# mcychan/nQuant.android

Hardware: NVIDIA B200
Metric: Mpixels/s 256-color PNN quantize+dither, 4K batch, 1/2/4/8 B200 vs JVM CPU (higher is better)
Workload: dtype f64

## Files before the change

### include/nquant_b200.h

```cpp
#ifndef NQUANT_B200_H
#define NQUANT_B200_H

#include <stdint.h>

#ifdef __cplusplus
extern "C" {
#endif

#define NQ_KIND_PNN 0
#define NQ_KIND_PNNLAB 1

#define NQ_OK 0
#define NQ_ERR_CUDA (-1)
#define NQ_ERR_ARG (-2)
#define NQ_ERR_COLOR (-3)
#define NQ_ERR_UNSUPPORTED (-4)
#define NQ_ERR_NOMEM (-5)

typedef struct nq_ctx nq_ctx;

int nq_device_count(void);

nq_ctx* nq_create(int device);
void nq_destroy(nq_ctx* ctx);
// ... 15 lines not shown
int nq_convert_batch_multi(nq_ctx** contexts, int n_contexts, int kind, const uint32_t* argb_in, int n_images, int width, int height,
                           int n_max_colors, int dither, const uint64_t* rng_seeds, uint32_t* argb_out, uint32_t* palettes_out,
                           int* palette_lens, int* has_alpha, int queue_images);

int nq_convert_batch_device(nq_ctx* ctx, int kind, const uint32_t* d_argb_in, int n_images, int width, int height,
                            int n_max_colors, int dither, const uint64_t* rng_seeds, uint32_t* d_argb_out,
                            uint32_t* palettes_out, int* palette_lens, int* has_alpha);

int nq_dither_with_palette(nq_ctx* ctx, int kind, const uint32_t* argb_in, int width, int height, int n_max_colors,
                           int dither, uint64_t rng_seed, const uint32_t* palette_in, int palette_len, uint32_t* argb_out);

int nq_histogram(nq_ctx* ctx, int kind, const uint32_t* argb_in, int width, int height, int n_max_colors, int* n_bins,
                 double* bins5, float* init_err, int* init_nn, int capacity);

int nq_gilbert_order(int width, int height, uint32_t* order_out);


typedef struct nq_image_info {
  int has_semi_transparency;
  int transparent_pixel_index;
  uint32_t transparent_color;
  int maxbins, quan_rt, texicab, is_nano;
  double weight, ratio_init, ratio_merge, pr, pg, pb, pa;
  int g_margin, g_thresold, g_dither_max_q, g_dither_max, g_sorted, g_has_alpha, g_use_saliency;
  float g_beta;
  float bn_weight;
  int palette_len;
  unsigned long long merges, rescans, pair_tests, rng_draws, heap_pops;
  int error;
  unsigned long long full_evals;
  unsigned long long merge_cycles[6], live_blocks, screened;
  unsigned long long dither_cycles[3];
  unsigned long long merge_rounds, rescans_discarded;
} nq_image_info;
int nq_get_image_info(nq_ctx* ctx, int image, nq_image_info* out);
int nq_sizeof_image_info(void);

int nq_set_spec_dither(nq_ctx* ctx, int on, int segment, int warmup);
int nq_get_spec_stats(nq_ctx* ctx, unsigned long long* images, unsigned long long* rounds, unsigned long long* fallbacks);

int nq_set_debug(nq_ctx* ctx, int flag);
int nq_debug_get_bins(nq_ctx* ctx, int image, double* bins5, float* init_err, int* init_nn);
int nq_debug_get_merges(nq_ctx* ctx, int image, int* pairs);
int nq_debug_get_saliencies(nq_ctx* ctx, int image, float* out);

unsigned long long nq_kernel_launches(nq_ctx* ctx);
int nq_get_stage_times(nq_ctx* ctx, double* ms, unsigned long long* launches, int reset);
int nq_get_kernel_times(nq_ctx* ctx, double* ms, unsigned long long* launches, int reset);
int nq_debug_math(nq_ctx* ctx, int fn, const double* x, const double* y, double* out, int n);

int nq_debug_ciede(nq_ctx* ctx, const float* lab1, const float* lab2, float* out, int* n_exact, int n);

int nq_synth_device(nq_ctx* ctx, uint32_t* d_out, int n_images, int width, int height, int cls, int alpha_mode,
                    uint64_t seed0);

#ifdef __cplusplus
}
#endif
#endif
```

### nquant_android_b200/_lib.py

```python
import ctypes
import os

HERE = os.path.dirname(os.path.abspath(__file__))
SO = os.path.join(HERE, "libnquant_b200.so")

SYMBOLS = [
    "nq_device_count", "nq_create", "nq_destroy", "nq_last_error", "nq_convert", "nq_convert_batch",
    "nq_convert_batch_device", "nq_dither_with_palette", "nq_gilbert_order", "nq_get_image_info", "nq_set_debug",
    "nq_debug_get_bins", "nq_debug_get_merges", "nq_debug_get_saliencies", "nq_kernel_launches", "nq_debug_math",
    "nq_synth_device", "nq_get_stage_times", "nq_set_stream", "nq_debug_ciede", "nq_sizeof_image_info",
    "nq_set_spec_dither", "nq_get_spec_stats", "nq_reset_stream", "nq_set_chunk_images", "nq_get_kernel_times", "nq_convert_batch_multi", "nq_histogram",
]

NQ_KIND_PNN, NQ_KIND_PNNLAB = 0, 1
NQ_OK, NQ_ERR_CUDA, NQ_ERR_ARG, NQ_ERR_COLOR, NQ_ERR_UNSUPPORTED, NQ_ERR_NOMEM = 0, -1, -2, -3, -4, -5


class ImageInfo(ctypes.Structure):
    _fields_ = [
        ("has_semi_transparency", ctypes.c_int), ("transparent_pixel_index", ctypes.c_int),
        ("transparent_color", ctypes.c_uint32),
        ("maxbins", ctypes.c_int), ("quan_rt", ctypes.c_int), ("texicab", ctypes.c_int), ("is_nano", ctypes.c_int),
        ("weight", ctypes.c_double), ("ratio_init", ctypes.c_double), ("ratio_merge", ctypes.c_double),
        ("pr", ctypes.c_double), ("pg", ctypes.c_double), ("pb", ctypes.c_double), ("pa", ctypes.c_double),
        ("g_margin", ctypes.c_int), ("g_thresold", ctypes.c_int), ("g_dither_max_q", ctypes.c_int),
        ("g_dither_max", ctypes.c_int), ("g_sorted", ctypes.c_int), ("g_has_alpha", ctypes.c_int),
        ("g_use_saliency", ctypes.c_int),
        ("g_beta", ctypes.c_float), ("bn_weight", ctypes.c_float), ("palette_len", ctypes.c_int),
        ("merges", ctypes.c_ulonglong), ("rescans", ctypes.c_ulonglong), ("pair_tests", ctypes.c_ulonglong),
        ("rng_draws", ctypes.c_ulonglong), ("heap_pops", ctypes.c_ulonglong),
        ("error", ctypes.c_int),
        ("full_evals", ctypes.c_ulonglong),
        ("merge_cycles", ctypes.c_ulonglong * 6), ("live_blocks", ctypes.c_ulonglong), ("screened", ctypes.c_ulonglong),
        ("dither_cycles", ctypes.c_ulonglong * 3),
        ("merge_rounds", ctypes.c_ulonglong), ("rescans_discarded", ctypes.c_ulonglong),
    ]

    def as_dict(self):
        return {n: (list(getattr(self, n)) if n in ("merge_cycles", "dither_cycles") else getattr(self, n)) for n, _ in self._fields_}


_lib = None


def load():
    global _lib
    if _lib is not None:
        return _lib
    if not os.path.exists(SO):
        raise ImportError(f"{SO} is missing: run `python -c 'import __graft_entry__ as g; g.build()'` "
                          "(nvcc, sm_100a). This package has no CPU fallback.")
    L = ctypes.CDLL(SO)
    vp, ci, u64 = ctypes.c_void_p, ctypes.c_int, ctypes.c_uint64
    L.nq_device_count.restype = ci
    L.nq_create.restype = vp
    L.nq_create.argtypes = [ci]
    L.nq_destroy.argtypes = [vp]
    L.nq_destroy.restype = None
    L.nq_last_error.restype = ctypes.c_char_p
    L.nq_convert.argtypes = [vp, ci, vp, ci, ci, ci, ci, u64, vp, vp, vp, vp]
    L.nq_convert_batch.argtypes = [vp, ci, vp, ci, ci, ci, ci, ci, vp, vp, vp, vp, vp]
    L.nq_convert_batch_device.argtypes = [vp, ci, vp, ci, ci, ci, ci, ci, vp, vp, vp, vp, vp]
    L.nq_convert_batch_multi.argtypes = [vp, ci, ci, vp, ci, ci, ci, ci, ci, vp, vp, vp, vp, vp, ci]
    L.nq_dither_with_palette.argtypes = [vp, ci, vp, ci, ci, ci, ci, u64, vp, ci, vp]
    L.nq_gilbert_order.argtypes = [ci, ci, vp]
    L.nq_histogram.argtypes = [vp, ci, vp, ci, ci, ci, vp, vp, vp, vp, ci]
    L.nq_get_image_info.argtypes = [vp, ci, vp]
    L.nq_set_debug.argtypes = [vp, ci]
# ... 22 lines not shown
```

### nquant_android_b200/csrc/nq_api.cu

```cuda
#include <cuda_runtime.h>
#include <stdint.h>
#include <stdio.h>
#include <stdlib.h>
#include <string.h>
#include <string>
#include <vector>
#include <map>
#include <utility>
#include <algorithm>
#include <mutex>
#include <thread>
#include <atomic>
#include <nvtx3/nvToolsExt.h>

#include "../../include/nquant_b200.h"
#include "nq_types.h"
#include "nq_math.h"
#include "nq_color.h"
#include "nq_bluenoise_table.h"
#include "nq_hist.cuh"
#include "nq_pnn.cuh"
#include "nq_dither.cuh"
#include "nq_dither_spec.cuh"

// ... 116 lines not shown
  out[4 * i] = tL; out[4 * i + 1] = tC; out[4 * i + 2] = tH; out[4 * i + 3] = tRT;
}

__global__ void k_set_palette(NqImage* imgs, int img, const uint32_t* pal, int plen) {
  if (threadIdx.x < plen) imgs[img].palette[threadIdx.x] = pal[threadIdx.x];
  if (threadIdx.x == 0) imgs[img].paletteLen = plen;
}

struct LabLutEntry { float4* ptr = nullptr; int refs = 0; };
std::mutex g_lutMutex;
std::map<int, LabLutEntry> g_lut;

struct DebugImage {
  std::vector<double> bins5;
  std::vector<float> initErr;
  std::vector<int> initNn;
  std::vector<int> merges;
  std::vector<float> sal;
};

}

#define NQ_FRONT_STREAMS 2
#define NQ_SPEC_BULK_DEFAULT 0

struct nq_ctx {
  int device = 0;
  cudaStream_t stream = nullptr;
  cudaStream_t ownStream = nullptr;
  cudaStream_t sFront[NQ_FRONT_STREAMS] = {}, sDith = nullptr, sAux = nullptr, sOut = nullptr, sIn = nullptr;
  std::vector<cudaEvent_t> evPool;
  size_t evUsed = 0;
  int smCount = 148;
  unsigned long long launches = 0;
  bool debug = false;
  int chunkImages = 0;
  std::map<std::pair<int, int>, uint32_t*> orders;
  std::vector<std::pair<int, int>> orderLru;
  size_t orderBytes = 0;
  unsigned char* ws = nullptr;
  size_t wsBytes = 0;
  NqImage* dImgs = nullptr;
  NqSlot* dSlots = nullptr;
  int* dLive = nullptr;
  int* dPos = nullptr;
  unsigned char* zeroPlane = nullptr;
  unsigned char* memoPlane = nullptr;
  unsigned char* sortPool = nullptr;
  size_t zeroSlotBytes = 0, memoSlotBytes = 0, sortSetBytes = 0, sortABytes = 0;
  int wsSlots = 0, wsNpix = 0, wsKind = -1, sortSets = 0;
  bool wsDebug = false, wsBits = false, wsIdx = false;
  std::vector<NqSlot> hSlots;
  uint32_t* dIn = nullptr;
  uint32_t* dOut = nullptr;
  size_t stageBytes = 0;
  double stageMs[NQ_NSTAGES] = {};
  unsigned long long stageLaunches[NQ_NSTAGES] = {};
  double kernelMs[NQ_NKERNELS] = {};
  unsigned long long kernelLaunches[NQ_NKERNELS] = {};
  bool specDither = true;
  int specSeg = 0, specWarm = 1024;
  size_t specPoolMaxBytes = 0;
  int specSlotsMax = 0;
  nq::spec::SpecImage* dSpec = nullptr;
  int specCap = 0;
  unsigned char* specBuf = nullptr;
// ... 127 lines not shown
  uint32_t* d = nullptr;
  CU(cudaMalloc(&d, bytes));
  cudaError_t e = cudaMemcpy(d, host.data(), bytes, cudaMemcpyHostToDevice);
  if (e != cudaSuccess) { cudaFree(d); return fail(NQ_ERR_CUDA, std::string("cudaMemcpy(order): ") + cudaGetErrorString(e)); }
  c->orders[key] = d;
  c->orderLru.push_back(key);
  c->orderBytes += bytes;
  *out = d;
  return NQ_OK;
}

int pixel_grid_x(const nq_ctx* c, int npix, int nimg) {
  int want = (npix + 256 * 8 - 1) / (256 * 8);
  int cap = std::max(1, (c->smCount * 8) / std::max(1, nimg));
  return std::max(1, std::min(want, cap));
}

cudaEvent_t take_event(nq_ctx* c) {
  if (c->evUsed == c->evPool.size()) {
    cudaEvent_t e = nullptr;
    cudaEventCreate(&e);
    c->evPool.push_back(e);
  }
  return c->evPool[c->evUsed++];
}

struct NvtxRange {
  explicit NvtxRange(const char* name) { nvtxRangePushA(name); }
  ~NvtxRange() { nvtxRangePop(); }
};

struct Chunk {
  int base = 0, n = 0;
  cudaStream_t front = nullptr;
  int frontIdx = 0;
  cudaEvent_t evIn = nullptr;
  cudaEvent_t ev[5] = {};
  cudaEvent_t evD[3] = {};
  cudaEvent_t evK[2 * NQ_NKERNELS] = {};
  std::vector<std::pair<cudaEvent_t, cudaEvent_t>> evRuns;
  unsigned long long launches[NQ_NSTAGES] = {};
  int copied = 0;
  uint32_t* hOut = nullptr;
  const uint32_t* dOut = nullptr;
  size_t imageBytes = 0;
};

struct SpecCudaBackend {
  nq_ctx* c;
  Chunk* ch;
  cudaStream_t st;
  bool timing = false;
  cudaEvent_t t0 = nullptr, t1 = nullptr;
  cudaError_t err = cudaSuccess;
  template <class... P, class... A>
  void launch(void (*kernel)(P...), dim3 grid, int block, A... args) {
    kernel<<<grid, block, 0, st>>>(args...);
    ++c->launches;
  }
  template <class... P, class... A>
  void launch_run(void (*kernel)(P...), dim3 grid, int block, A... args) {
    cudaEvent_t a = take_event(c), b = take_event(c);
    cudaEventRecord(a, st);
    kernel<<<grid, block, 0, st>>>(args...);
    cudaEventRecord(b, st);
    ch->evRuns.emplace_back(a, b);
// ... 84 lines not shown
  for (int i = 0; i < n; ++i) plan->any += (elig[i] & 255) == 1;
  plan->seg = seg; plan->nslots = nslots;
  return NQ_OK;
}
int spec_rounds(nq_ctx* c, Chunk& ch, cudaStream_t st, int npix, const SpecPlan& plan, const std::vector<int>& elig, std::vector<int>& handed) {
  using namespace nq::spec;
  handed.clear();
  if (!plan.any) return NQ_OK;
  SpecCudaBackend be{c, &ch, st};
  be.timing = getenv("NQ_SPEC_TIMING") != nullptr;
  be.begin();
  SpecStats stats;
  handed.assign(plan.any, 0);
  spec_drive(be, c->dImgs + ch.base, c->dSpec + ch.base, c->dSpecPool, elig.data(), ch.n, npix, plan.seg, plan.nslots, c->dSpecInts, c->dTanh,
             c->smCount, &stats, handed.data());
  handed.resize((size_t)stats.handedBack);
  be.end();
  c->specImages += stats.done; c->specRounds += stats.rounds; c->specFallbacks += stats.handedBack;
  CU(be.err);
  CU(cudaGetLastError());
  return NQ_OK;
}

struct GroupArgs {
  int kind, w, h, nmax, dither;
  const uint64_t* seeds;
  const uint32_t* dPalIn;
  int palInLen;
  const uint32_t* hIn;
  uint32_t* hOut;
  bool stopAfterSweep = false;
};

int enqueue_front(nq_ctx* c, Chunk& ch, const GroupArgs& A, const uint32_t* dIn, uint32_t* dOut) {
  NvtxRange nv("nq front (scan, histogram, find_nn, merge)");
  const int n = ch.n, npix = A.w * A.h, kind = A.kind, nmax = A.nmax;
  cudaStream_t st = ch.front;
  NqImage* dI = c->dImgs + ch.base;
  NqSlot* dS = c->dSlots + ch.base;
  if (ch.evIn) CU(cudaStreamWaitEvent(st, ch.evIn, 0));
  std::vector<NqImage> hImgs(n);
  for (int i = 0; i < n; ++i) {
    NqImage& I = hImgs[i];
    memset(&I, 0, sizeof(I));
    I.kind = kind; I.width = A.w; I.height = A.h; I.npix = npix; I.nmax = nmax; I.dither = A.dither;
    I.seed = A.seeds ? A.seeds[ch.base + i] : 0ULL;
    I.transIdx = -1;
    NqSlot& S = c->hSlots[ch.base + i];
    S.in = dIn + (size_t)(ch.base + i) * npix;
    S.out = dOut + (size_t)(ch.base + i) * npix;
    if (kind == NQ_KIND_LAB) {
      unsigned char* sp = c->sortPool + c->sortSetBytes * ((size_t)ch.frontIdx * c->sortSets + (size_t)(i % c->sortSets));
      S.sortA = reinterpret_cast<uint32_t*>(sp);
      S.sortB = reinterpret_cast<uint32_t*>(sp + c->sortABytes);
      S.warpHist = reinterpret_cast<unsigned int*>(sp + 2 * c->sortABytes);
    }
  }
  CU(cudaMemcpyAsync(dI, hImgs.data(), sizeof(NqImage) * n, cudaMemcpyHostToDevice, st));
  CU(cudaMemcpyAsync(dS, c->hSlots.data() + ch.base, sizeof(NqSlot) * n, cudaMemcpyHostToDevice, st));
  CU(cudaMemsetAsync(c->zeroPlane + c->zeroSlotBytes * ch.base, 0, c->zeroSlotBytes * n, st));
  CU(cudaMemsetAsync(c->memoPlane + c->memoSlotBytes * ch.base, 0xFF, c->memoSlotBytes * n, st));
  for (int i = 0; i < n; ++i) if (c->hSlots[ch.base + i].bits) CU(cudaMemsetAsync(c->hSlots[ch.base + i].bits, 0, (size_t)1 << 29, st));
  const int gx = pixel_grid_x(c, npix, n);
  const dim3 pg(gx, n);
  unsigned long long l0 = c->launches;
  auto mark = [&](int k) { cudaEventRecord(ch.ev[k], st); if (k > 0) { ch.launches[k - 1] += c->launches - l0; l0 = c->launches; } };
  mark(0);
  nq::k_alpha_scan<<<pg, 256, 0, st>>>(dI, dS); ++c->launches;
  nq::k_setup_scan<<<(n + 127) / 128, 128, 0, st>>>(dI, dS, n); ++c->launches;
  mark(1);
  if (nmax > 2) {
    if (kind == NQ_KIND_RGB) {
      {
        const int ntiles = ((A.w + NQ_HTW - 1) / NQ_HTW) * ((A.h + NQ_HTW - 1) / NQ_HTW);
        const dim3 hg(std::max(1, std::min(ntiles, std::max(1, c->smCount * 8 / n))), n);
        nq::k_hist_rgb<<<hg, 256, sizeof(nq::HistTable), st>>>(dI, dS); ++c->launches;
      }
      nq::k_finalize_rgb<<<n, 1024, 0, st>>>(dI, dS); ++c->launches;
    } else {
      const int nruns = (npix + NQ_RUN - 1) / NQ_RUN;
// ... 30 lines not shown
      std::vector<NqImage> tmp(n);
      CU(cudaMemcpy(tmp.data(), dI, sizeof(NqImage) * n, cudaMemcpyDeviceToHost));
      for (int i = 0; i < n; ++i) {
        DebugImage& D = c->dbg[ch.base + i];
        const int mb = tmp[i].maxbins;
        const NqSlot& S = c->hSlots[ch.base + i];
        D.bins5.assign((size_t)mb * 5, 0.0);
        D.initErr.assign(mb, 0.f); D.initNn.assign(mb, 0);
        if (mb <= 0) continue;
        std::vector<double> col(mb);
        std::vector<float> colf(mb);
        for (int k = 0; k < 4; ++k) {
          if (kind == NQ_KIND_RGB) {
            const double* src = k == 0 ? S.bAc : k == 1 ? S.bC1 : k == 2 ? S.bC2 : S.bC3;
            CU(cudaMemcpy(col.data(), src, (size_t)mb * 8, cudaMemcpyDeviceToHost));
          } else {
            const float* src = k == 0 ? S.fAc : k == 1 ? S.fC1 : k == 2 ? S.fC2 : S.fC3;
            CU(cudaMemcpy(colf.data(), src, (size_t)mb * 4, cudaMemcpyDeviceToHost));
            for (int b = 0; b < mb; ++b) col[b] = colf[b];
          }
          for (int b = 0; b < mb; ++b) D.bins5[(size_t)b * 5 + k] = col[b];
        }
        CU(cudaMemcpy(colf.data(), S.bCnt, (size_t)mb * 4, cudaMemcpyDeviceToHost));
        for (int b = 0; b < mb; ++b) D.bins5[(size_t)b * 5 + 4] = colf[b];
        CU(cudaMemcpy(D.initErr.data(), S.bErr, (size_t)mb * 4, cudaMemcpyDeviceToHost));
        CU(cudaMemcpy(D.initNn.data(), S.bNn, (size_t)mb * 4, cudaMemcpyDeviceToHost));
      }
    }
    if (A.stopAfterSweep) { mark(4); CU(cudaGetLastError()); return NQ_OK; }
    int* live = c->dLive + (size_t)ch.base * NQ_NBINS;
    int* pos = c->dPos + (size_t)ch.base * NQ_NBINS;
    if (kind == NQ_KIND_RGB) {
      nq::k_merge_rgb<<<n, NQ_RGB_THREADS, (size_t)NQ_RGB_HEAP_SMEM * 8, st>>>(dI, dS, live, pos, c->debug ? 1 : 0); ++c->launches;
    } else {
      nq::k_merge_lab<<<n, NQ_LAB_THREADS, (size_t)NQ_LAB_HEAP_SMEM * 8, st>>>(dI, dS, live, pos, c->debug ? 1 : 0); ++c->launches;
    }
  } else { mark(2); mark(3); }
  mark(4);
  CU(cudaGetLastError());
  return NQ_OK;
}

int run_dither(nq_ctx* c, Chunk& ch, const GroupArgs& A, const uint32_t* dOrder) {
  NvtxRange nv("nq dither (setup, Gilbert pass, BlueNoise pass)");
  const int n = ch.n, npix = A.w * A.h, kind = A.kind;
  cudaStream_t st = c->sDith, ax = c->sAux;
  NqImage* dI = c->dImgs + ch.base;
  NqSlot* dS = c->dSlots + ch.base;
  unsigned long long l0 = c->launches;
  CU(cudaStreamWaitEvent(st, ch.ev[4], 0));
  CU(cudaEventRecord(ch.evD[0], st));
  nq::k_dither_setup<<<(n + 63) / 64, 64, 0, st>>>(dI, dS, n); ++c->launches;
  if (A.dPalIn) {
    for (int i = 0; i < n; ++i) { k_set_palette<<<1, 256, 0, st>>>(dI, i, A.dPalIn, A.palInLen); ++c->launches; }
    nq::k_dither_setup<<<(n + 63) / 64, 64, 0, st>>>(dI, dS, n); ++c->launches;
  }
  const dim3 pg(pixel_grid_x(c, npix, n), n);
  if (kind == NQ_KIND_LAB && c->debug) { nq::k_saliency<<<pg, 256, 0, st>>>(dI, dS); ++c->launches; }
  if (kind == NQ_KIND_LAB) { nq::k_build_cells<<<dim3(std::max(1, std::min(128, c->smCount * 8 / n)), n), 256, 0, st>>>(dI, dS); ++c->launches; }
  CU(cudaEventRecord(ch.evD[1], st));
  ch.launches[4] += c->launches - l0; l0 = c->launches;
  std::vector<int> elig, handed;
  const bool spec = c->specDither && kind == NQ_KIND_LAB && A.dither;
  SpecPlan plan;
  if (spec) {
    int rc = spec_prepare(c, ch, st, npix, dOrder, elig, &plan);
    if (rc) return rc;
  }
// ... 34 lines not shown
}

int check_args(nq_ctx* c, int kind, const void* in, int n, int w, int h, int nmax, const void* out) {
  if (!c) return fail(NQ_ERR_ARG, "null context");
  if (kind != NQ_KIND_PNN && kind != NQ_KIND_PNNLAB) return fail(NQ_ERR_ARG, "kind must be NQ_KIND_PNN or NQ_KIND_PNNLAB");
  if (!in || !out) return fail(NQ_ERR_ARG, "null pixel buffer");
  if (n <= 0 || w <= 0 || h <= 0) return fail(NQ_ERR_ARG, "n_images, width and height must be positive");
  if ((long long)w * h > 0x7fffffffLL / 4) return fail(NQ_ERR_ARG, "image too large");
  if (nmax < 2) return fail(NQ_ERR_ARG, "n_max_colors must be >= 2 (the reference indexes palette[1], PnnQuantizer.java:446)");
  if (nmax > NQ_MAXK) return fail(NQ_ERR_UNSUPPORTED, "n_max_colors > 256 is not supported by this build");
  return NQ_OK;
}

int collect_results(nq_ctx* c, int base, int n, uint32_t* palettes, int* plens, int* hasAlpha, int* firstErr) {
  for (int i = 0; i < n; ++i) {
    const NqImage& I = c->lastImgs[i];
    if (palettes) memcpy(palettes + (size_t)(base + i) * NQ_MAXK, I.palette, sizeof(uint32_t) * NQ_MAXK);
    if (plens) plens[base + i] = I.paletteLen;
    if (hasAlpha) hasAlpha[base + i] = I.transIdx > -1;
    if (I.error && !*firstErr) *firstErr = I.error;
  }
  return NQ_OK;
}

int convert_group(nq_ctx* c, const GroupArgs& A, int n, const uint32_t* dIn, uint32_t* dOut, int dbgBase) {
  const int npix = A.w * A.h;
  const uint32_t* dOrder = nullptr;
  int rc = ensure_order(c, A.w, A.h, &dOrder);
  if (rc) return rc;
  std::vector<int> sizes;
  if (c->debug) sizes.push_back(n);
  else if (c->chunkImages > 0) { for (int b = 0; b < n; b += c->chunkImages) sizes.push_back(std::min(c->chunkImages, n - b)); }
  else {
    const int pieces = std::max(n <= 640 ? 1 : (n + 511) / 512, (A.hIn && n >= 32) ? 2 : 1);
    for (int k = 0; k < pieces; ++k) sizes.push_back(n / pieces + (k < n % pieces ? 1 : 0));
  }
  const int nch = (int)sizes.size();
  c->evUsed = 0;
  std::vector<Chunk> chunks(nch);
  cudaEvent_t evStart = take_event(c), evOut = take_event(c), evEnd = take_event(c);
  CU(cudaEventRecord(evStart, c->stream));
  for (int k = 0; k < NQ_FRONT_STREAMS; ++k) CU(cudaStreamWaitEvent(c->sFront[k], evStart, 0));
  CU(cudaStreamWaitEvent(c->sDith, evStart, 0));
  CU(cudaStreamWaitEvent(c->sOut, evStart, 0));
  CU(cudaStreamWaitEvent(c->sIn, evStart, 0));
  for (int k = 0, base = 0; k < nch; base += sizes[k], ++k) {
    Chunk& ch = chunks[k];
    ch.base = base; ch.n = sizes[k];
    ch.frontIdx = k % NQ_FRONT_STREAMS; ch.front = c->sFront[ch.frontIdx];
    for (auto& e : ch.ev) e = take_event(c);
    for (auto& e : ch.evD) e = take_event(c);
    if (A.hIn) {
      ch.evIn = take_event(c);
      CU(cudaMemcpyAsync(const_cast<uint32_t*>(dIn) + (size_t)ch.base * npix, A.hIn + (size_t)ch.base * npix, (size_t)ch.n * npix * 4, cudaMemcpyHostToDevice, c->sIn));
      CU(cudaEventRecord(ch.evIn, c->sIn));
    }
  }
  if (c->debug) for (int i = 0; i < n; ++i) c->dbg[dbgBase + i] = DebugImage{};
  GroupArgs G = A;
  for (int k = 0; k < nch; ++k) { rc = enqueue_front(c, chunks[k], G, dIn, dOut); if (rc) return rc; }
  for (int k = 0; k < nch; ++k) {
    if (A.stopAfterSweep) {
      CU(cudaStreamWaitEvent(c->sDith, chunks[k].ev[4], 0));
      for (auto& e : chunks[k].evD) CU(cudaEventRecord(e, c->sDith));
      continue;
    }
    if (A.hOut) { chunks[k].hOut = A.hOut + (size_t)chunks[k].base * npix; chunks[k].dOut = dOut + (size_t)chunks[k].base * npix; chunks[k].imageBytes = (size_t)npix * 4; }
    rc = run_dither(c, chunks[k], G, dOrder);
    if (rc) return rc;
    if (A.hOut && chunks[k].copied < chunks[k].n) {
      Chunk& ch = chunks[k];
      CU(cudaStreamWaitEvent(c->sOut, ch.evD[2], 0));
      CU(cudaMemcpyAsync(A.hOut + (size_t)(ch.base + ch.copied) * npix, dOut + (size_t)(ch.base + ch.copied) * npix, (size_t)(ch.n - ch.copied) * npix * 4,
                         cudaMemcpyDeviceToHost, c->sOut));
    }
  }
  CU(cudaEventRecord(evOut, c->sOut));
  CU(cudaStreamWaitEvent(c->sDith, evOut, 0));
  c->lastImgs.resize(n);
  CU(cudaMemcpyAsync(c->lastImgs.data(), c->dImgs, sizeof(NqImage) * n, cudaMemcpyDeviceToHost, c->sDith));
  CU(cudaEventRecord(evEnd, c->sDith));
// ... 156 lines not shown
  if (const char* e = getenv("NQ_SPEC_SLOTS")) c->specSlotsMax = atoi(e);
  if (const char* e = getenv("NQ_SPEC_POOL_GB")) c->specPoolMaxBytes = (size_t)atoi(e) << 30;
  bool haveLut = false;
  {
    DevBuf dBn, dW;
    ok = dBn.alloc(4096) == cudaSuccess && cudaMemcpy(dBn.p, kBlueNoise, 4096, cudaMemcpyHostToDevice) == cudaSuccess &&
         dW.alloc(sizeof(float) * 3 * (NQ_MAXQ + 3)) == cudaSuccess && cudaMalloc(&c->dTanh, sizeof(float) * 512) == cudaSuccess;
    if (ok) {
      nq::k_init_tables<<<4, 256, 0, c->stream>>>(dBn.as<signed char>()); ++c->launches;
      nq::k_init_rtfac<<<1, 256, 0, c->stream>>>(); ++c->launches;
      k_spec_tables<<<2, 256, 0, c->stream>>>(c->dTanh, dW.as<float>()); ++c->launches;
      ok = cudaMemcpyToSymbolAsync(nq::spec::c_specW, dW.p, sizeof(float) * 3 * (NQ_MAXQ + 3), 0, cudaMemcpyDeviceToDevice, c->stream) == cudaSuccess &&
           cudaStreamSynchronize(c->stream) == cudaSuccess;
    }
  }
  if (ok) {
    std::lock_guard<std::mutex> lk(g_lutMutex);
    LabLutEntry& e = g_lut[device];
    if (!e.ptr) {
      ok = cudaMalloc(&e.ptr, sizeof(float4) << 24) == cudaSuccess;
      if (ok) {
        nq::k_build_lab_lut<<<65536, 256, 0, c->stream>>>(e.ptr); ++c->launches;
        const float4* cp = e.ptr;
        ok = cudaMemcpyToSymbolAsync(nq::g_labLut, &cp, sizeof(cp), 0, cudaMemcpyHostToDevice, c->stream) == cudaSuccess &&
             cudaStreamSynchronize(c->stream) == cudaSuccess;
      }
      if (!ok && e.ptr) { cudaFree(e.ptr); e.ptr = nullptr; }
    }
    if (ok) { ++e.refs; haveLut = true; }
  }
  if (ok) ok = cudaFuncSetAttribute(nq::k_merge_rgb, cudaFuncAttributeMaxDynamicSharedMemorySize, NQ_RGB_HEAP_SMEM * 8) == cudaSuccess;
  if (ok) ok = cudaFuncSetAttribute(nq::k_hist_rgb, cudaFuncAttributeMaxDynamicSharedMemorySize, (int)sizeof(nq::HistTable)) == cudaSuccess;
  if (ok) ok = cudaFuncSetAttribute(nq::k_dither_fifo, cudaFuncAttributeMaxDynamicSharedMemorySize, 32768) == cudaSuccess;
  if (ok) ok = cudaFuncSetAttribute(nq::k_merge_lab, cudaFuncAttributeMaxDynamicSharedMemorySize, NQ_LAB_HEAP_SMEM * 8) == cudaSuccess;
  if (!ok) {
    fail(NQ_ERR_CUDA, std::string("context initialisation failed: ") + cudaGetErrorString(cudaGetLastError()));
    destroy_ctx(c, haveLut);
    return nullptr;
  }
  return c;
}

void nq_destroy(nq_ctx* c) {
  if (!c) return;
  destroy_ctx(c, true);
}

int nq_convert_batch_device(nq_ctx* c, int kind, const uint32_t* d_in, int n, int w, int h, int nmax, int dither,
                            const uint64_t* seeds, uint32_t* d_out, uint32_t* palettes, int* plens, int* hasAlpha) {
  int rc = check_args(c, kind, d_in, n, w, h, nmax, d_out);
  if (rc) return rc;
  NvtxRange nv("nq_convert_batch_device");
  return convert_device(c, kind, d_in, n, w, h, nmax, dither, seeds, d_out, palettes, plens, hasAlpha, nullptr, 0);
}

int nq_convert_batch(nq_ctx* c, int kind, const uint32_t* in, int n, int w, int h, int nmax, int dither, const uint64_t* seeds,
                     uint32_t* out, uint32_t* palettes, int* plens, int* hasAlpha) {
  int rc = check_args(c, kind, in, n, w, h, nmax, out);
  if (rc) return rc;
  NvtxRange nv("nq_convert_batch");
  CU(cudaSetDevice(c->device));
  const size_t bytes = (size_t)n * w * h * 4;
  rc = ensure_stage(c, bytes);
  if (rc) return rc;
  rc = convert_device(c, kind, c->dIn, n, w, h, nmax, dither, seeds, c->dOut, palettes, plens, hasAlpha, nullptr, 0, in, out);
  if (rc) return rc;
  CU(cudaStreamSynchronize(c->stream));
// ... 77 lines not shown
  const int mb = (int)D.initErr.size();
  *nBins = mb;
  if (mb > capacity && (bins5 || initErr || initNn)) return fail(NQ_ERR_ARG, "capacity is smaller than the number of occupied bins (call with null outputs to size them)");
  if (bins5) memcpy(bins5, D.bins5.data(), D.bins5.size() * 8);
  if (initErr) memcpy(initErr, D.initErr.data(), D.initErr.size() * 4);
  if (initNn) memcpy(initNn, D.initNn.data(), D.initNn.size() * 4);
  return NQ_OK;
}

int nq_gilbert_order(int w, int h, uint32_t* out) {
  if (w <= 0 || h <= 0 || !out) return fail(NQ_ERR_ARG, "bad arguments");
  size_t n = 0;
  gilbert_walk(w, h, [&](int x, int y) { out[n++] = (uint32_t)(x + y * w); });
  return n == (size_t)w * h ? NQ_OK : fail(NQ_ERR_ARG, "gilbert walk size mismatch");
}

int nq_get_image_info(nq_ctx* c, int image, nq_image_info* o) {
  if (!c || !o || image < 0 || image >= (int)c->lastImgs.size()) return fail(NQ_ERR_ARG, "no such image in the last batch");
  const NqImage& I = c->lastImgs[image];
  memset(o, 0, sizeof(*o));
  o->has_semi_transparency = I.hasSemi; o->transparent_pixel_index = I.transIdx; o->transparent_color = I.transColor;
  o->maxbins = I.maxbins; o->quan_rt = I.quan_rt; o->texicab = I.texicab; o->is_nano = I.isNano;
  o->weight = I.weight; o->ratio_init = I.ratio; o->ratio_merge = I.ratioMerge;
  o->pr = I.PR; o->pg = I.PG; o->pb = I.PB; o->pa = I.PA;
  o->g_margin = I.gMargin; o->g_thresold = I.gThresold; o->g_dither_max_q = I.gDitherMaxQ; o->g_dither_max = I.gDitherMax;
  o->g_sorted = I.gSorted; o->g_has_alpha = I.gHasAlpha; o->g_use_saliency = I.gUseSal; o->g_beta = I.gBeta;
  o->bn_weight = I.bnWeight; o->palette_len = I.paletteLen;
  o->merges = (I.nmax > 2 && I.extbins > 0) ? (unsigned long long)I.extbins : 0ULL;
  o->rescans = I.statRescans; o->pair_tests = I.statPairs; o->rng_draws = I.rngDraws; o->heap_pops = I.statHeapPops;
  o->full_evals = I.statFullEvals;
  for (int k = 0; k < 6; ++k) o->merge_cycles[k] = I.statCyc[k];
  o->live_blocks = I.statLiveBlocks; o->screened = I.statScreened;
  o->merge_rounds = I.statRounds; o->rescans_discarded = I.statDiscarded;
  for (int k = 0; k < 3; ++k) o->dither_cycles[k] = I.statDither[k];
  o->error = I.error;
  return NQ_OK;
}

int nq_sizeof_image_info(void) { return (int)sizeof(nq_image_info); }

int nq_set_stream(nq_ctx* c, void* stream) {
  if (!c) return fail(NQ_ERR_ARG, "null context");
  c->stream = stream ? reinterpret_cast<cudaStream_t>(stream) : cudaStreamLegacy;
  return NQ_OK;
}
int nq_reset_stream(nq_ctx* c) {
  if (!c) return fail(NQ_ERR_ARG, "null context");
  c->stream = c->ownStream;
  return NQ_OK;
}
int nq_set_chunk_images(nq_ctx* c, int images) {
  if (!c || images < 0) return fail(NQ_ERR_ARG, "bad arguments");
  c->chunkImages = images;
  return NQ_OK;
}

int nq_set_spec_dither(nq_ctx* c, int on, int segment, int warmup) {
  if (!c) return fail(NQ_ERR_ARG, "null context");
  if (on && ((segment != 0 && segment < 64) || warmup < 0 || warmup > (1 << 24))) return fail(NQ_ERR_ARG, "segment must be 0 (automatic) or >= 64 pixels, warm-up >= 0");
  c->specDither = on != 0;
  if (on) { c->specSeg = segment; c->specWarm = warmup; }
  return NQ_OK;
}
int nq_get_spec_stats(nq_ctx* c, unsigned long long* images, unsigned long long* rounds, unsigned long long* fallbacks) {
  if (!c) return fail(NQ_ERR_ARG, "null context");
  if (images) *images = c->specImages;
// ... 100 lines not shown
```

### nquant_android_b200/csrc/nq_pnn.cuh

```cuda
#pragma once
#include "nq_types.h"
#include "nq_color.h"
#include "nq_hist.cuh"
#include "nq_fastmath.cuh"

namespace nq {

__device__ const float c_coeffs[3][3] = {{0.299f, 0.587f, 0.114f}, {-0.14713f, -0.28886f, 0.436f}, {0.615f, -0.51499f, -0.10001f}};

struct RgbProbe {
  float n1;
  double wa, wr, wg, wb;
  double PR, PG, PB, PA, ratio;
  int start;
  bool semi;
};

__device__ __forceinline__ RgbProbe rgb_probe(const NqImage& I, const NqSlot& S, int idx) {
  RgbProbe P;
  P.n1 = S.bCnt[idx];
  P.wa = S.bAc[idx]; P.wr = S.bC1[idx]; P.wg = S.bC2[idx]; P.wb = S.bC3[idx];
  P.PR = I.PR; P.PG = I.PG; P.PB = I.PB; P.PA = I.PA; P.ratio = I.ratio;
  P.semi = I.hasSemi != 0;
  P.start = 0;
// ... 340 lines not shown
template <int HS>
struct HeapView {
  static_assert((HS & 1) == 0, "children l2, l2 + 1 must fall on the same side of the split");
  float* sErr; unsigned* sIdNn;
  uint2* gH;
  __device__ __forceinline__ float err(int l) const { return l < HS ? sErr[l] : __uint_as_float(gH[l].x); }
  __device__ __forceinline__ unsigned idnn(int l) const { return l < HS ? sIdNn[l] : gH[l].y; }
  __device__ __forceinline__ int id(int l) const { return (int)(idnn(l) & 0xFFFFu); }
  __device__ __forceinline__ void set(int l, unsigned idnn_, float e) {
    if (l < HS) { sErr[l] = e; sIdNn[l] = idnn_; } else gH[l] = make_uint2(__float_as_uint(e), idnn_);
  }
  __device__ __forceinline__ void sift_down(unsigned idnn1, float e1, int heapN) {
    int l = 1, l2;
    for (; (l2 = l + l) <= heapN; l = l2) {
      float ea, eb = 0.f;
      unsigned ia, ib = 0u;
      if (l2 < HS) {
        ea = sErr[l2]; ia = sIdNn[l2];
        if (l2 < heapN) { eb = sErr[l2 + 1]; ib = sIdNn[l2 + 1]; }
      } else {
        const uint4 ch = *reinterpret_cast<const uint4*>(&gH[l2]);
        ea = __uint_as_float(ch.x); ia = ch.y; eb = __uint_as_float(ch.z); ib = ch.w;
      }
      if (l2 < heapN && ea > eb) { ++l2; ea = eb; ia = ib; }
      if (e1 <= ea) break;
      set(l, ia, ea);
    }
    set(l, idnn1, e1);
  }
};
__device__ __forceinline__ unsigned pack_idnn(int id, int nn) { return (unsigned)id | ((unsigned)nn << 16); }

#define NQ_LAB_THREADS 128
#define NQ_LAB_HEAP_SMEM 5632
#define NQ_LAB_ROUND 4

__device__ __forceinline__ int block_excl_scan_128(int v, int* total, int* sScan ) {
  const unsigned lane = lane_id(), w = threadIdx.x >> 5;
  int x = v;
#pragma unroll
  for (int o = 1; o < 32; o <<= 1) {
    int y = __shfl_up_sync(0xffffffffu, x, o);
    if (lane >= (unsigned)o) x += y;
  }
  if (lane == 31) sScan[w] = x;
  __syncthreads();
  int base = 0, tot = 0;
#pragma unroll
  for (int k = 0; k < NQ_LAB_THREADS / 32; ++k) { const int c = sScan[k]; if (k < (int)w) base += c; tot += c; }
  *total = tot;
  __syncthreads();
  return base + x - v;
}

__device__ __forceinline__ int rebuild_live_lab(const NqSlot& S, const LabScratch& X, int maxbins, int* live, int* posOf, int* sScan) {
  const int t = threadIdx.x;
  const unsigned lane = lane_id(), w = t >> 5;
  const int W = NQ_LAB_THREADS / 32;
  const int per = (((maxbins + W - 1) / W) + 31) & ~31;
  const int b0 = min(maxbins, (int)w * per), b1 = min(maxbins, b0 + per);
  int c = 0;
  for (int b = b0 + (int)lane; b < b1; b += 32) c += S.bMtm[b] != NQ_DELETED;
  int total, j = block_excl_scan_128(c, &total, sScan);
  j = __shfl_sync(0xffffffffu, j, 0);
  for (int base = b0; base < b1; base += 32) {
    const int b = base + (int)lane;
    const bool alive = b < b1 && S.bMtm[b] != NQ_DELETED;
    const unsigned m = __ballot_sync(0xffffffffu, alive);
    if (alive) {
      const int p = j + __popc(m & ((1u << lane) - 1u));
      live[p] = b; posOf[b] = p;
      X.q[p] = make_float4(S.bCnt[b], S.fC1[b], S.fC2[b], S.fC3[b]);
      X.al[p] = S.fAc[b];
    }
    j += __popc(m);
  }
  __syncthreads();
  const int nblk = (total + 31) >> 5;
  for (int blk = t; blk < nblk; blk += NQ_LAB_THREADS) lab_block_summary(X.q, total, blk, X.bs);
  __syncthreads();
  return total;
}

__global__ void __launch_bounds__(NQ_LAB_THREADS, 4) k_merge_lab(NqImage* imgs, const NqSlot* slots, int* liveBuf, int* posBuf, int logMerges) {
  constexpr int R = NQ_LAB_ROUND;
  static_assert(R >= 1 && 32 * R <= NQ_LAB_THREADS, "a batch holds 32 blocks of each bin of the round, one per thread");
  extern __shared__ unsigned char smemRaw[];
  float* sErr = reinterpret_cast<float*>(smemRaw);
  unsigned* sId = reinterpret_cast<unsigned*>(smemRaw + (size_t)NQ_LAB_HEAP_SMEM * 4);
  __shared__ int sScan[8];
  __shared__ unsigned sBits[R][64];
  __shared__ unsigned short sPre[R][65];
  __shared__ unsigned short sBat[NQ_LAB_THREADS];
  __shared__ unsigned sMaskA[NQ_LAB_THREADS];
  __shared__ unsigned sMaskB[NQ_LAB_THREADS];
  __shared__ int sOffA[NQ_LAB_THREADS + 1], sOffB[NQ_LAB_THREADS];
  __shared__ double sGs[NQ_LAB_THREADS], sGw[NQ_LAB_THREADS], sF[NQ_LAB_THREADS];
  __shared__ int sPos[NQ_LAB_THREADS];
  __shared__ LabProbe sProbe[R];
  __shared__ double sErrR[R];
  __shared__ int sBinR[R], sNnR[R], sFirstR[R];
  __shared__ int sAction, sB1, sHeapN, sIter, sNRound;

  const int img = blockIdx.x;
  NqImage& I = imgs[img];
  if (I.kind != NQ_KIND_LAB || I.nmax <= 2 || I.skipPnn) return;
  const NqSlot& S = slots[img];
  const LabScratch X = lab_scratch(S);
  const int t = threadIdx.x;
  const unsigned lane = lane_id(), w = t >> 5;
  const int W = NQ_LAB_THREADS / 32;
  const int maxbins = I.maxbins, extbins = I.extbins;
  int* live = liveBuf + (size_t)img * NQ_NBINS;
  int* posOf = posBuf + (size_t)img * NQ_NBINS;
  HeapView<NQ_LAB_HEAP_SMEM> H{sErr, sId, S.heap};
  const float4 dead = make_float4(-1.f, 0.f, 0.f, 0.f);

  if (w == 0) {
    int heapN = 0;
    for (int base = 0; base < maxbins; base += 32) {
      float e = (base + (int)lane < maxbins) ? S.bErr[base + lane] : 0.f;
      const int nnv = (base + (int)lane < maxbins) ? S.bNn[base + lane] : 0;
      const int cnt = min(32, maxbins - base);
      for (int j = 0; j < cnt; ++j) {
        const float err = __shfl_sync(0xffffffffu, e, j);
        const int nnj = __shfl_sync(0xffffffffu, nnv, j);
        int l = ++heapN, l2;
        for (; l > 1; l = l2) {
          l2 = l >> 1;
          float pe = H.err(l2);
          if (pe <= err) break;
          unsigned pid = H.idnn(l2);
          if (lane == 0) H.set(l, pid, pe);
        }
        if (lane == 0) H.set(l, pack_idnn(base + j, nnj), err);
        __syncwarp();
      }
    }
    if (lane == 0) { sHeapN = heapN; sIter = 0; sNRound = 0; }
  }
  __syncthreads();
  int liveLen = rebuild_live_lab(S, X, maxbins, live, posOf, sScan);
  int liveAtRebuild = liveLen, iterAtRebuild = 0;
  unsigned long long rescans = 0, pairs = 0, fulls = 0, liveBlocks = 0, screened = 0, rounds = 0, discarded = 0;
  unsigned pops = 0;
  unsigned used = 0;
  const double ratioMerge = I.ratioMerge;
  long long cyc[6] = {0, 0, 0, 0, 0, 0};
// ... 703 lines not shown
```

### nquant_android_b200/csrc/nq_types.h

```cpp
#pragma once
#include <stdint.h>

#define NQ_MAXK 256
#define NQ_NBINS 65536
#define NQ_DELETED 0xFFFF
#define NQ_MAXQ 25

enum NqKind { NQ_KIND_RGB = 0, NQ_KIND_LAB = 1 };

struct NqImage {
  int kind, width, height, npix, nmax, dither;
  unsigned long long seed;
  unsigned int semiCount;
  int transIdx;
  int hasSemi;
  uint32_t transColor;
  int fixA0;
  int keyTransp;
  int maxbins, extbins, quan_rt, texicab, isNano, skipPnn;
  double PR, PG, PB, PA, ratio, ratioMerge, weight;
  int paletteLen;
  uint32_t palette[NQ_MAXK];
  int gMargin, gThresold, gDitherMaxQ , gDitherMax, gSorted, gHasAlpha, gUseSal;
  float gBeta;
  double gWeight;
  float gWeights[NQ_MAXQ];
  float gW1[1], gW3[3], gW7[7];
  float bnWeight;
  int error;
  unsigned long long statRescans, statPairs, rngDraws, statFullEvals;
  unsigned int statHeapPops;
  unsigned int distinctColors;
  unsigned long long statCyc[6], statLiveBlocks, statScreened;
  unsigned long long statRounds, statDiscarded;
  unsigned long long statDither[3];
  int specDone;
  unsigned int nonOpaque;
  int bnParallel;
  int pad1;
};

struct NqSlot {
  const uint32_t* in;
  uint32_t* out;
  unsigned int* hCnt;
  unsigned long long* hSum;
  unsigned int* keyOff;
  uint32_t* sortA;
  uint32_t* sortB;
  unsigned int* warpHist;
  float* sal;
  double* bAc; double* bC1; double* bC2; double* bC3;
  float* fAc; float* fC1; float* fC2; float* fC3;
  float* bCnt; float* bErr;
  int* bNn; int* bTm; int* bMtm;
  uint2* heap;
  int* mergeLog;
  unsigned short* memo;
  unsigned short* idx;
  unsigned char* cells;
  unsigned int* bits;
};
```

Before: 777.9.

## Template LAB merge kernel on CTAs per SM and size chunks from occupancy

Turns the LAB PNN merge kernel into a template over the target CTAs per SM. The 8-CTA variant uses a smaller shared-memory heap (2048 entries instead of 5632), and it is chosen when the merge work in flight would exceed the SMs' capacity at 4 CTAs each. Chunk sizes now come from the occupancy API (SM count times resident merge CTAs) instead of the fixed 512/640 thresholds. The aim is to fit more images' merges on the GPU at once, at the cost of more heap spills to global memory and tighter register limits in the 8-CTA variant.

```diff
diff --git a/include/nquant_b200.h b/include/nquant_b200.h
--- a/include/nquant_b200.h
+++ b/include/nquant_b200.h
@@ -71,6 +71,7 @@
   unsigned long long merge_cycles[6], live_blocks, screened;
   unsigned long long dither_cycles[3];
   unsigned long long merge_rounds, rescans_discarded;
+  int merge_ctas_per_sm;
 } nq_image_info;
 int nq_get_image_info(nq_ctx* ctx, int image, nq_image_info* out);
 int nq_sizeof_image_info(void);
diff --git a/nquant_android_b200/_lib.py b/nquant_android_b200/_lib.py
--- a/nquant_android_b200/_lib.py
+++ b/nquant_android_b200/_lib.py
@@ -34,6 +34,7 @@
         ("merge_cycles", ctypes.c_ulonglong * 6), ("live_blocks", ctypes.c_ulonglong), ("screened", ctypes.c_ulonglong),
         ("dither_cycles", ctypes.c_ulonglong * 3),
         ("merge_rounds", ctypes.c_ulonglong), ("rescans_discarded", ctypes.c_ulonglong),
+        ("merge_ctas_per_sm", ctypes.c_int),
     ]
 
     def as_dict(self):
diff --git a/nquant_android_b200/csrc/nq_api.cu b/nquant_android_b200/csrc/nq_api.cu
--- a/nquant_android_b200/csrc/nq_api.cu
+++ b/nquant_android_b200/csrc/nq_api.cu
@@ -172,6 +172,7 @@
   std::vector<cudaEvent_t> evPool;
   size_t evUsed = 0;
   int smCount = 148;
+  int mergeLab4PerSm = 0, mergeLab8PerSm = 0, mergeRgbPerSm = 0;
   unsigned long long launches = 0;
   bool debug = false;
   int chunkImages = 0;
@@ -365,6 +366,7 @@
 
 struct Chunk {
   int base = 0, n = 0;
+  int mergeInFlight = 0;
   cudaStream_t front = nullptr;
   int frontIdx = 0;
   cudaEvent_t evIn = nullptr;
@@ -515,6 +517,8 @@
   bool stopAfterSweep = false;
 };
 
+int lab_merge_ctas(const nq_ctx* c, const Chunk& ch) { return ch.mergeInFlight > c->smCount * c->mergeLab4PerSm ? 8 : 4; }
+
 int enqueue_front(nq_ctx* c, Chunk& ch, const GroupArgs& A, const uint32_t* dIn, uint32_t* dOut) {
   NvtxRange nv("nq front (scan, histogram, find_nn, merge)");
   const int n = ch.n, npix = A.w * A.h, kind = A.kind, nmax = A.nmax;
@@ -529,6 +533,7 @@
     I.kind = kind; I.width = A.w; I.height = A.h; I.npix = npix; I.nmax = nmax; I.dither = A.dither;
     I.seed = A.seeds ? A.seeds[ch.base + i] : 0ULL;
     I.transIdx = -1;
+    I.mergeCtas = kind == NQ_KIND_LAB ? (lab_merge_ctas(c, ch) == 8 ? c->mergeLab8PerSm : c->mergeLab4PerSm) : c->mergeRgbPerSm;
     NqSlot& S = c->hSlots[ch.base + i];
     S.in = dIn + (size_t)(ch.base + i) * npix;
     S.out = dOut + (size_t)(ch.base + i) * npix;
@@ -625,8 +630,10 @@
     int* pos = c->dPos + (size_t)ch.base * NQ_NBINS;
     if (kind == NQ_KIND_RGB) {
       nq::k_merge_rgb<<<n, NQ_RGB_THREADS, (size_t)NQ_RGB_HEAP_SMEM * 8, st>>>(dI, dS, live, pos, c->debug ? 1 : 0); ++c->launches;
+    } else if (lab_merge_ctas(c, ch) == 8) {
+      nq::k_merge_lab<8><<<n, NQ_LAB_THREADS, (size_t)nq::lab_heap_smem(8) * 8, st>>>(dI, dS, live, pos, c->debug ? 1 : 0); ++c->launches;
     } else {
-      nq::k_merge_lab<<<n, NQ_LAB_THREADS, (size_t)NQ_LAB_HEAP_SMEM * 8, st>>>(dI, dS, live, pos, c->debug ? 1 : 0); ++c->launches;
+      nq::k_merge_lab<4><<<n, NQ_LAB_THREADS, (size_t)nq::lab_heap_smem(4) * 8, st>>>(dI, dS, live, pos, c->debug ? 1 : 0); ++c->launches;
     }
   } else { mark(2); mark(3); }
   mark(4);
@@ -727,7 +734,8 @@
   if (c->debug) sizes.push_back(n);
   else if (c->chunkImages > 0) { for (int b = 0; b < n; b += c->chunkImages) sizes.push_back(std::min(c->chunkImages, n - b)); }
   else {
-    const int pieces = std::max(n <= 640 ? 1 : (n + 511) / 512, (A.hIn && n >= 32) ? 2 : 1);
+    const int slots = c->smCount * (A.kind == NQ_KIND_LAB ? c->mergeLab8PerSm : c->mergeRgbPerSm);
+    const int pieces = std::max((n + slots - 1) / slots, (A.hIn && n >= 32) ? 2 : 1);
     for (int k = 0; k < pieces; ++k) sizes.push_back(n / pieces + (k < n % pieces ? 1 : 0));
   }
   const int nch = (int)sizes.size();
@@ -742,6 +750,7 @@
   for (int k = 0, base = 0; k < nch; base += sizes[k], ++k) {
     Chunk& ch = chunks[k];
     ch.base = base; ch.n = sizes[k];
+    ch.mergeInFlight = sizes[k] + std::max(k > 0 ? sizes[k - 1] : 0, k + 1 < nch ? sizes[k + 1] : 0);
     ch.frontIdx = k % NQ_FRONT_STREAMS; ch.front = c->sFront[ch.frontIdx];
     for (auto& e : ch.ev) e = take_event(c);
     for (auto& e : ch.evD) e = take_event(c);
@@ -964,7 +973,12 @@
   if (ok) ok = cudaFuncSetAttribute(nq::k_merge_rgb, cudaFuncAttributeMaxDynamicSharedMemorySize, NQ_RGB_HEAP_SMEM * 8) == cudaSuccess;
   if (ok) ok = cudaFuncSetAttribute(nq::k_hist_rgb, cudaFuncAttributeMaxDynamicSharedMemorySize, (int)sizeof(nq::HistTable)) == cudaSuccess;
   if (ok) ok = cudaFuncSetAttribute(nq::k_dither_fifo, cudaFuncAttributeMaxDynamicSharedMemorySize, 32768) == cudaSuccess;
-  if (ok) ok = cudaFuncSetAttribute(nq::k_merge_lab, cudaFuncAttributeMaxDynamicSharedMemorySize, NQ_LAB_HEAP_SMEM * 8) == cudaSuccess;
+  if (ok) ok = cudaFuncSetAttribute(nq::k_merge_lab<4>, cudaFuncAttributeMaxDynamicSharedMemorySize, nq::lab_heap_smem(4) * 8) == cudaSuccess &&
+               cudaFuncSetAttribute(nq::k_merge_lab<8>, cudaFuncAttributeMaxDynamicSharedMemorySize, nq::lab_heap_smem(8) * 8) == cudaSuccess;
+  if (ok) ok = cudaOccupancyMaxActiveBlocksPerMultiprocessor(&c->mergeLab4PerSm, nq::k_merge_lab<4>, NQ_LAB_THREADS, nq::lab_heap_smem(4) * 8) == cudaSuccess &&
+               cudaOccupancyMaxActiveBlocksPerMultiprocessor(&c->mergeLab8PerSm, nq::k_merge_lab<8>, NQ_LAB_THREADS, nq::lab_heap_smem(8) * 8) == cudaSuccess &&
+               cudaOccupancyMaxActiveBlocksPerMultiprocessor(&c->mergeRgbPerSm, nq::k_merge_rgb, NQ_RGB_THREADS, NQ_RGB_HEAP_SMEM * 8) == cudaSuccess &&
+               c->mergeLab4PerSm > 0 && c->mergeLab8PerSm > 0 && c->mergeRgbPerSm > 0;
   if (!ok) {
     fail(NQ_ERR_CUDA, std::string("context initialisation failed: ") + cudaGetErrorString(cudaGetLastError()));
     destroy_ctx(c, haveLut);
@@ -1108,6 +1122,7 @@
   for (int k = 0; k < 6; ++k) o->merge_cycles[k] = I.statCyc[k];
   o->live_blocks = I.statLiveBlocks; o->screened = I.statScreened;
   o->merge_rounds = I.statRounds; o->rescans_discarded = I.statDiscarded;
+  o->merge_ctas_per_sm = I.mergeCtas;
   for (int k = 0; k < 3; ++k) o->dither_cycles[k] = I.statDither[k];
   o->error = I.error;
   return NQ_OK;
diff --git a/nquant_android_b200/csrc/nq_pnn.cuh b/nquant_android_b200/csrc/nq_pnn.cuh
--- a/nquant_android_b200/csrc/nq_pnn.cuh
+++ b/nquant_android_b200/csrc/nq_pnn.cuh
@@ -396,7 +396,7 @@
 __device__ __forceinline__ unsigned pack_idnn(int id, int nn) { return (unsigned)id | ((unsigned)nn << 16); }
 
 #define NQ_LAB_THREADS 128
-#define NQ_LAB_HEAP_SMEM 5632
+__host__ __device__ constexpr int lab_heap_smem(int ctas) { return ctas >= 8 ? 2048 : 5632; }
 #define NQ_LAB_ROUND 4
 
 __device__ __forceinline__ int block_excl_scan_128(int v, int* total, int* sScan ) {
@@ -446,12 +446,13 @@
   return total;
 }
 
-__global__ void __launch_bounds__(NQ_LAB_THREADS, 4) k_merge_lab(NqImage* imgs, const NqSlot* slots, int* liveBuf, int* posBuf, int logMerges) {
-  constexpr int R = NQ_LAB_ROUND;
+template <int CTAS>
+__global__ void __launch_bounds__(NQ_LAB_THREADS, CTAS) k_merge_lab(NqImage* imgs, const NqSlot* slots, int* liveBuf, int* posBuf, int logMerges) {
+  constexpr int R = NQ_LAB_ROUND, HS = lab_heap_smem(CTAS);
   static_assert(R >= 1 && 32 * R <= NQ_LAB_THREADS, "a batch holds 32 blocks of each bin of the round, one per thread");
   extern __shared__ unsigned char smemRaw[];
   float* sErr = reinterpret_cast<float*>(smemRaw);
-  unsigned* sId = reinterpret_cast<unsigned*>(smemRaw + (size_t)NQ_LAB_HEAP_SMEM * 4);
+  unsigned* sId = reinterpret_cast<unsigned*>(smemRaw + (size_t)HS * 4);
   __shared__ int sScan[8];
   __shared__ unsigned sBits[R][64];
   __shared__ unsigned short sPre[R][65];
@@ -477,7 +478,7 @@
   const int maxbins = I.maxbins, extbins = I.extbins;
   int* live = liveBuf + (size_t)img * NQ_NBINS;
   int* posOf = posBuf + (size_t)img * NQ_NBINS;
-  HeapView<NQ_LAB_HEAP_SMEM> H{sErr, sId, S.heap};
+  HeapView<HS> H{sErr, sId, S.heap};
   const float4 dead = make_float4(-1.f, 0.f, 0.f, 0.f);
 
   if (w == 0) {
diff --git a/nquant_android_b200/csrc/nq_types.h b/nquant_android_b200/csrc/nq_types.h
--- a/nquant_android_b200/csrc/nq_types.h
+++ b/nquant_android_b200/csrc/nq_types.h
@@ -33,6 +33,7 @@
   unsigned int distinctColors;
   unsigned long long statCyc[6], statLiveBlocks, statScreened;
   unsigned long long statRounds, statDiscarded;
+  int mergeCtas;
   unsigned long long statDither[3];
   int specDone;
   unsigned int nonOpaque;
```

After: 828.9, median of 6. 1.07x the previous value.
